# zixinz990/quadruped_landing

Measured on AMD Instinct MI355X. Metric: knot-point constraint+Jacobian evals/sec, higher is better.
Workload: dtype f64

## Files before the change

include/qln_evaluator.h:

```cpp
#ifndef QLN_EVALUATOR_H
#define QLN_EVALUATOR_H

#include <stdint.h>

#ifdef __cplusplus
extern "C" {
#endif

#define QLN_NX 15
#define QLN_NU 5
#define QLN_NZ 20
#define QLN_COST_STRIDE 41

#define QLN_OK 0
#define QLN_ERR_INVALID_ARGUMENT (-1)
#define QLN_ERR_HIP (-2)
#define QLN_ERR_NO_DEVICE (-3)
#define QLN_ERR_UNSUPPORTED (-4)

#define QLN_JAC_WRITE_CONSTANTS 1u

#define QLN_JAC_FORMAT_DENSE_BLOCKS 0
#define QLN_JAC_FORMAT_STRUCTURAL 1

// ... 118 lines not shown
                             const double* K_dot, const double* x0_dot, double* Zout_dot);
int qln_tracking_rollout_jvp_host(qln_handle* h, const double* Zref, const double* K, const double* Zout,
                                  const double* Zref_dot, const double* K_dot, const double* x0_dot, double* Zout_dot);
#define QLN_TRACK_MARG_STRIDE 8
int qln_tracking_covariance(qln_handle* h, const double* Zout, const double* K, const double* Sigma0, int32_t sigma0_batch,
                            const double* Wdiag, double* Sigma, double* marg);
int qln_tracking_covariance_host(qln_handle* h, const double* Zout, const double* K, const double* Sigma0,
                                 int32_t sigma0_batch, const double* Wdiag, double* Sigma, double* marg);
int qln_perturb_point(qln_handle* h, const qln_drop_state_sampler* s, double* Z, double sigma, double h_min, double h_max,
                      int redraw_h);
int qln_get_boundary_states(qln_handle* h, double* x0, double* xf);
int qln_set_lqr_cost(qln_handle* h, const double* Qdiag, const double* Rdiag, const double* Qfdiag, double dt,
                     int per_problem);
int qln_get_cost(qln_handle* h, double* cost_host, int32_t* cost_batch);

int qln_eval_objective_host(qln_handle* h, const double* Z, double* f);
int qln_eval_objective_gradient_host(qln_handle* h, const double* Z, double* grad);
int qln_eval_constraint_host(qln_handle* h, const double* Z, double* c);
int qln_eval_constraint_jacobian_host(qln_handle* h, const double* Z, double* vals);
int qln_eval_hessian_lagrangian_host(qln_handle* h, const double* Z, const double* sigma, const double* mu, double* hvals);
int qln_eval_hessian_lagrangian_product_host(qln_handle* h, const double* Z, const double* sigma, const double* mu,
                                             const double* v, double* y);
int qln_eval_constraint_jvp_host(qln_handle* h, const double* Z, const double* v, double* y);
int qln_eval_constraint_vjp_host(qln_handle* h, const double* Z, const double* lam, double* g);
int qln_eval_constraint_jacobian_dense_host(qln_handle* h, int32_t b, const double* Z, double* jac);

int qln_vals_alloc_placed(qln_handle* h, const double* Z, double* c, double** vals, float* ms_best);
int qln_vals_alloc_placed_budget(qln_handle* h, const double* Z, double* c, int64_t transient_bytes, double** vals, float* ms_best);
int qln_vals_placed_address_space(int64_t* retired_bytes, int64_t* cap_bytes);
int qln_vals_free_placed(qln_handle* h, double* vals);
int qln_vals_placed_info(const qln_handle* h, const double* vals, int64_t* chunk_bytes, int64_t* chunks_scanned,
                         int64_t* window_first_chunk);

int qln_time_constraint_and_jacobian(qln_handle* h, const double* Z, double* c, double* vals, uint32_t flags,
                                     int32_t warmup, int32_t iters, float* ms_each );
int qln_time_constraint_and_jacobian_total(qln_handle* h, const double* Z, double* c, double* vals, uint32_t flags,
                                           int32_t warmup, int32_t iters, float* ms_total);

#ifdef __cplusplus
}
#endif
#endif
```

quadruped_landing_amd/_lib.py:

```python
from __future__ import annotations

import ctypes as C
import os

_HERE = os.path.dirname(os.path.abspath(__file__))
LIB_PATH = os.environ.get("QLN_LIB_PATH") or os.path.join(_HERE, "csrc", "libqln_hip.so")

QLN_OK = 0
QLN_ERR_INVALID_ARGUMENT = -1
QLN_ERR_HIP = -2
QLN_ERR_NO_DEVICE = -3
QLN_ERR_UNSUPPORTED = -4
QLN_JAC_WRITE_CONSTANTS = 1
QLN_JAC_FORMAT_DENSE_BLOCKS = 0
QLN_JAC_FORMAT_STRUCTURAL = 1

NX, NU, NZ, COST_STRIDE = 15, 5, 20, 41
GN_INFO_STRIDE = 8
HESS_STEP_NNZ, HESS_TERM_NNZ = 55, 15
TRACK_NU, TRACK_P_NNZ = 4, 120
TRACK_MARG_STRIDE = 8


class QlnModel(C.Structure):
    _fields_ = [(n, C.c_double) for n in ("g", "mb", "mf", "lb", "l1", "l2")]


class QlnBatchDesc(C.Structure):
    _fields_ = [
        ("B", C.c_int32),
        ("N", C.c_int32),
        ("model", QlnModel),
        ("k_trans", C.POINTER(C.c_int32)),
        ("init_mode", C.POINTER(C.c_int32)),
        ("x0", C.POINTER(C.c_double)),
        ("xf", C.POINTER(C.c_double)),
        ("cost", C.POINTER(C.c_double)),
        ("cost_batch", C.c_int32),
        ("z_stride", C.c_int64),
        ("align", C.c_int32),
        ("jac_format", C.c_int32),
    ]


class QlnDims(C.Structure):
    _fields_ = [
# ... 98 lines not shown
    "qln_tracking_rollout_jvp": (C.c_int, [_vp, _dp, _dp, _dp, _dp, _dp, _dp, _dp]),
    "qln_tracking_rollout_jvp_host": (C.c_int, [_vp, _dp, _dp, _dp, _dp, _dp, _dp, _dp]),
    "qln_tracking_covariance": (C.c_int, [_vp, _dp, _dp, _dp, C.c_int32, _dp, _dp, _dp]),
    "qln_tracking_covariance_host": (C.c_int, [_vp, _dp, _dp, _dp, C.c_int32, _dp, _dp, _dp]),
    "qln_eval_constraint_jvp_host": (C.c_int, [_vp, _dp, _dp, _dp]),
    "qln_eval_constraint_vjp_host": (C.c_int, [_vp, _dp, _dp, _dp]),
    "qln_gauss_newton_step": (C.c_int, [_vp, _dp, _dp, _dp, C.c_int32, C.c_double, _dp, _dp, _dp]),
    "qln_eval_kinematic_constraint": (C.c_int, [_vp, _dp, _dp, _dp]),
    "qln_kinematic_bounds": (C.c_int, [_vp, C.POINTER(C.c_double), C.POINTER(C.c_double)]),
    "qln_eval_friction_cone": (C.c_int, [_vp, _dp, C.c_double, _dp, _dp]),
    "qln_constraint_violation": (C.c_int, [_vp, _dp, _dp]),
    "qln_solve_default_options": (C.c_int, [C.POINTER(QlnSolveOptions)]),
    "qln_variable_bounds": (C.c_int, [C.c_int32, C.POINTER(QlnSolveOptions), _dp, _dp]),
    "qln_solve": (C.c_int, [_vp, _dp, C.POINTER(QlnSolveOptions), _dp]),
    "qln_solve_host": (C.c_int, [_vp, _dp, C.POINTER(QlnSolveOptions), _dp]),
    "qln_initial_guess": (C.c_int, [_vp, _dp]),
    "qln_sample_drop_states": (C.c_int, [_vp, C.POINTER(QlnDropStateSampler)]),
    "qln_sample_bounded_integers": (C.c_int, [C.c_int, C.POINTER(C.c_uint64), C.POINTER(C.c_uint64), C.c_int64, C.c_int32, C.c_int32, C.c_int64,
                                            _i32p, _i64p]),
    "qln_perturb_point": (C.c_int, [_vp, C.POINTER(QlnDropStateSampler), _dp, C.c_double, C.c_double, C.c_double, C.c_int]),
    "qln_get_boundary_states": (C.c_int, [_vp, _dp, _dp]),
    "qln_set_lqr_cost": (C.c_int, [_vp, _dp, _dp, _dp, C.c_double, C.c_int]),
    "qln_get_cost": (C.c_int, [_vp, _dp, _i32p]),
    "qln_eval_objective_host": (C.c_int, [_vp, _dp, _dp]),
    "qln_eval_objective_gradient_host": (C.c_int, [_vp, _dp, _dp]),
    "qln_eval_constraint_host": (C.c_int, [_vp, _dp, _dp]),
    "qln_eval_constraint_jacobian_host": (C.c_int, [_vp, _dp, _dp]),
    "qln_eval_constraint_jacobian_dense_host": (C.c_int, [_vp, C.c_int32, _dp, _dp]),
    "qln_vals_alloc_placed": (C.c_int, [_vp, _dp, _dp, C.POINTER(_vp), C.POINTER(C.c_float)]),
    "qln_vals_free_placed": (C.c_int, [_vp, _dp]),
    "qln_vals_alloc_placed_budget": (C.c_int, [_vp, _dp, _dp, C.c_int64, C.POINTER(_vp), C.POINTER(C.c_float)]),
    "qln_vals_placed_address_space": (C.c_int, [_i64p, _i64p]),
    "qln_vals_placed_info": (C.c_int, [_vp, _dp, _i64p, _i64p, _i64p]),
    "qln_time_constraint_and_jacobian": (C.c_int, [_vp, _dp, _dp, _dp, C.c_uint32, C.c_int32, C.c_int32, C.POINTER(C.c_float)]),
    "qln_time_constraint_and_jacobian_total": (C.c_int, [_vp, _dp, _dp, _dp, C.c_uint32, C.c_int32, C.c_int32, C.POINTER(C.c_float)]),
}


def lib() -> C.CDLL:
    global _lib
    if _lib is None:
        if not os.path.exists(LIB_PATH) and not os.environ.get("QLN_LIB_PATH"):
            import shutil
            import subprocess

            csrc = os.path.join(_HERE, "csrc")
            if shutil.which("hipcc") or os.path.exists("/opt/rocm/bin/hipcc"):
                subprocess.call(["make", "-C", csrc, "libqln_hip.so"], stdout=subprocess.DEVNULL)
        if not os.path.exists(LIB_PATH):
            raise ImportError(
                f"{LIB_PATH} not found: build it with `make -C quadruped_landing_amd/csrc` "
                "(hipcc --offload-arch=gfx950).  There is no CPU fallback."
            )
        import torch

        L = C.CDLL(LIB_PATH)
        for name, (res, args) in SIGNATURES.items():
            fn = getattr(L, name)
            fn.restype = res
            fn.argtypes = args
        _lib = L
    return _lib


def check(rc: int) -> None:
    if rc != QLN_OK:
# ... 2 lines not shown
```

quadruped_landing_amd/csrc/qln_api.cpp:

```cpp
#include <hip/hip_runtime.h>

#include <algorithm>
#include <atomic>
#include <cmath>
#include <cstdio>
#include <cstdlib>
#include <cstring>
#include <initializer_list>
#include <limits>
#include <new>
#include <string>
#include <vector>

#include "../../include/qln_evaluator.h"
#include "qln_device.h"
#include "qln_hessian.h"

namespace {

thread_local std::string g_err;

int fail(int code, const std::string& msg) {
    g_err = msg;
    return code;
}

#define QLN_HIP(expr)                                                                                   \
    do {                                                                                                \
        hipError_t e_ = (expr);                                                                         \
        if (e_ != hipSuccess)                                                                           \
            return fail(QLN_ERR_HIP, std::string(#expr) + ": " + hipGetErrorString(e_));                \
    } while (0)

int64_t round_up(int64_t v, int64_t a) { return (v + a - 1) / a * a; }

int32_t hessian_nnz(int32_t N) { return QLN_HESS_STEP_NNZ * (N - 1) + QLN_HESS_TERM_NNZ; }
int64_t hessian_stride(int32_t N, int32_t align) { return round_up(hessian_nnz(N), align ? align : 16); }

constexpr bool kReturnVirtualRange = false;
constexpr uint64_t kVaCapBytes = (uint64_t)64 << 40;
std::atomic<uint64_t> g_va_retired{0};

int32_t m_nlp_of(int32_t N, int32_t kt) { return qln::row_layout(N, kt).m; }
int32_t nnz_dyn_of(int32_t N, int32_t kt, int32_t fmt) { return qln::vals_layout(N, kt, fmt).o_const; }
int32_t nnz_of(int32_t N, int32_t kt, int32_t fmt) { return qln::vals_layout(N, kt, fmt).nnz; }

int64_t tracking_k_total(const qln_dims& D) { return (int64_t)D.B * (D.N - 1) * QLN_TRACK_NU * QLN_NX; }
int64_t tracking_p_total(const qln_dims& D) { return (int64_t)D.B * D.N * QLN_TRACK_P_NNZ; }
int64_t tracking_marg_total(const qln_dims& D) { return (int64_t)D.B * D.N * QLN_TRACK_MARG_STRIDE; }

enum HostRole {
    kZ,
    kV,
    kZbar,
    kZio,
    kZdot,
    kZout,
    kGrad,
    kC,
    kMu,
    kVals,
    kF,
    kSigma,
    kHvals,
    kK,
    kKbar,
    kKdot,
    kP,
    kX0,
    kCov0,
    kCov,
    kMarg,
    kHostRoles
};

}

struct qln_handle {
    int device = 0;
    qln_model model{};
    hipStream_t stream = nullptr;
    qln::BatchParams p{};
    qln_dims dims{};
    std::vector<int32_t> k_trans, init_mode;
    std::vector<int64_t> c_off, j_off;
    qln::ProblemDesc* d_desc = nullptr;
    double* d_bnd = nullptr;
    double* d_cost = nullptr;
    int64_t h_stride = 0;
    double* staged[kHostRoles] = {};
    struct Mapped {
        double* host = nullptr;
        double* dev = nullptr;
    };
    Mapped mapped[kHostRoles];
    bool zero_copy = false;
    std::vector<double> h_vals_one;
    struct DenseMap {
        std::vector<int64_t> at, zeros;
    };
    std::vector<DenseMap> dense_map;
    struct Placed {
        char* va = nullptr;
        size_t va_size = 0;
        size_t chunk = 0;
        size_t first = 0;
        size_t scanned = 0;
        std::vector<hipMemGenericAllocationHandle_t> chunks;
        double* vals = nullptr;
    };
    std::vector<Placed> placed;
    double* solve_scratch = nullptr;
    size_t solve_scratch_n = 0;
};

namespace {

template <class T>
int upload(T** dst, const T* src, size_t n) {
    QLN_HIP(hipMalloc(reinterpret_cast<void**>(dst), std::max<size_t>(n, 1) * sizeof(T)));
    if (n) QLN_HIP(hipMemcpy(*dst, src, n * sizeof(T), hipMemcpyHostToDevice));
    return QLN_OK;
}

int64_t host_role_size(const qln_handle* h, HostRole r) {
    const qln_dims& D = h->dims;
    switch (r) {
        case kZ: case kV: case kZbar: case kZio: case kZdot: case kZout: case kGrad: return D.z_total;
        case kC: case kMu: return D.c_total;
        case kVals: return D.j_total;
        case kF: case kSigma: return D.B;
        case kHvals: return (int64_t)(D.B - 1) * h->h_stride + hessian_nnz(D.N);
        case kK: case kKbar: case kKdot: return tracking_k_total(D);
        case kP: case kCov: return tracking_p_total(D);
        case kCov0: return (int64_t)D.B * QLN_TRACK_P_NNZ;
        case kMarg: return tracking_marg_total(D);
        case kX0: return (int64_t)D.B * QLN_NX;
        case kHostRoles: break;
    }
    return 0;
}

int acquire(qln_handle* h, HostRole r, bool mapped) {
    const size_t bytes = std::max<int64_t>(host_role_size(h, r), 1) * sizeof(double);
// ... 190 lines not shown
    P.lb = d->model.lb;
    P.desc = h->d_desc;
    P.bnd = h->d_bnd;
    P.cost = h->d_cost;
    P.cost_batch = d->cost_batch;
    P.z_stride = z_stride;
    P.jac_format = fmt;
    P.kt_max = *std::max_element(d->k_trans, d->k_trans + d->B);
    h->zero_copy = (D.z_total + D.c_total + D.j_total) * (int64_t)sizeof(double) <= ((int64_t)8 << 20);
    *out = h;
    return QLN_OK;
}

static int release_placed(qln_handle::Placed& p) {
    hipError_t first = hipSuccess;
    const char* what = nullptr;
    auto note = [&](hipError_t e, const char* w) {
        if (e != hipSuccess && first == hipSuccess) {
            first = e;
            what = w;
        }
    };
    for (size_t i = 0; i < p.chunks.size(); ++i) {
        note(hipMemUnmap(p.va + (p.first + i) * p.chunk, p.chunk), "hipMemUnmap");
        note(hipMemRelease(p.chunks[i]), "hipMemRelease");
    }
    p.chunks.clear();
    if (p.va && kReturnVirtualRange) note(hipMemAddressFree(p.va, p.va_size), "hipMemAddressFree");
    p.va = nullptr;
    if (first != hipSuccess) return fail(QLN_ERR_HIP, std::string("releasing a placed buffer: ") + what + ": " + hipGetErrorString(first));
    return QLN_OK;
}

int qln_destroy(qln_handle* h) {
    if (!h) return QLN_OK;
    (void)hipSetDevice(h->device);
    int rc = QLN_OK;
    if (!h->placed.empty()) {
        if (hipError_t e = hipDeviceSynchronize(); e != hipSuccess)
            rc = fail(QLN_ERR_HIP, std::string("qln_destroy: hipDeviceSynchronize: ") + hipGetErrorString(e));
        for (auto& p : h->placed)
            if (int r = release_placed(p); r != QLN_OK && rc == QLN_OK) rc = r;
    }
    for (const qln_handle::Mapped& m : h->mapped)
        if (m.host) (void)hipHostFree(m.host);
    for (double* b : h->staged)
        if (b) (void)hipFree(b);
    void* bufs[] = {h->d_desc, h->d_bnd, h->d_cost, h->solve_scratch};
    for (void* b : bufs)
        if (b) (void)hipFree(b);
    delete h;
    return rc;
}

int qln_set_stream(qln_handle* h, void* hip_stream) {
    if (int rc = check_handle(h)) return rc;
    h->stream = reinterpret_cast<hipStream_t>(hip_stream);
    return QLN_OK;
}

int qln_synchronize(qln_handle* h) {
    if (int rc = check_handle(h)) return rc;
    if (int rc = bind_device(h)) return rc;
    QLN_HIP(hipStreamSynchronize(h->stream));
    return QLN_OK;
}

int qln_get_dims(const qln_handle* h, qln_dims* out) {
    if (int rc = check_handle(h)) return rc;
    if (!out) return fail(QLN_ERR_INVALID_ARGUMENT, "qln_get_dims: null out");
    *out = h->dims;
    return QLN_OK;
}

int qln_get_offsets(const qln_handle* h, int64_t* c_off, int64_t* j_off) {
// ... 881 lines not shown

static int time_fused(qln_handle* h, const double* Z, double* c, double* vals, int warmup, int iters, float* best) {
    hipEvent_t e0 = nullptr, e1 = nullptr;
    if (hipEventCreate(&e0) != hipSuccess || hipEventCreate(&e1) != hipSuccess) {
        if (e0) (void)hipEventDestroy(e0);
        return fail(QLN_ERR_HIP, "hipEventCreate failed");
    }
    int rc = QLN_OK;
    *best = 1e30f;
    for (int i = 0; i < warmup + iters && rc == QLN_OK; ++i) {
        (void)hipEventRecord(e0, h->stream);
        if (qln::launch_constraint_jacobian(h->p, 0, h->p.B, Z, c, vals, 0, h->stream) != hipSuccess) rc = fail(QLN_ERR_HIP, "launch failed");
        (void)hipEventRecord(e1, h->stream);
        if (rc == QLN_OK && hipEventSynchronize(e1) != hipSuccess) rc = fail(QLN_ERR_HIP, "hipEventSynchronize failed");
        float ms = 0.f;
        if (rc == QLN_OK && hipEventElapsedTime(&ms, e0, e1) != hipSuccess) rc = fail(QLN_ERR_HIP, "hipEventElapsedTime failed");
        if (rc == QLN_OK && i >= warmup) *best = std::min(*best, ms);
    }
    (void)hipEventDestroy(e0);
    (void)hipEventDestroy(e1);
    return rc;
}

int qln_vals_alloc_placed(qln_handle* h, const double* Z, double* c, double** vals, float* ms_best) {
    return qln_vals_alloc_placed_budget(h, Z, c, (int64_t)64 << 30, vals, ms_best);
}

int qln_vals_placed_address_space(int64_t* retired_bytes, int64_t* cap_bytes) {
    if (retired_bytes) *retired_bytes = (int64_t)g_va_retired.load();
    if (cap_bytes) *cap_bytes = (int64_t)kVaCapBytes;
    return QLN_OK;
}

int qln_vals_alloc_placed_budget(qln_handle* h, const double* Z, double* c, int64_t transient_bytes, double** vals, float* ms_best) {
    if (int rc = check_handle(h)) return rc;
    if (!Z || !vals) return fail(QLN_ERR_INVALID_ARGUMENT, "qln_vals_alloc_placed: null pointer");
    if (transient_bytes < 0) return fail(QLN_ERR_INVALID_ARGUMENT, "qln_vals_alloc_placed: negative transient budget");
    *vals = nullptr;
    if (int rc = bind_device(h)) return rc;
    hipMemAllocationProp prop = {};
    prop.type = hipMemAllocationTypePinned;
    prop.location.type = hipMemLocationTypeDevice;
    prop.location.id = h->device;
    size_t gran = 0;
    QLN_HIP(hipMemGetAllocationGranularity(&gran, &prop, hipMemAllocationGranularityRecommended));
    const size_t chunk = round_up((int64_t)256 << 20, (int64_t)gran);
    const size_t bytes = (size_t)h->dims.j_total * 8;
    const size_t need = (bytes + chunk - 1) / chunk;
    const size_t region = ((size_t)32 << 30) / chunk;
    const bool small = bytes < ((size_t)1 << 30);
    size_t free_b = 0, total_b = 0;
    QLN_HIP(hipMemGetInfo(&free_b, &total_b));
    const size_t budget = free_b / 10 * 9 / chunk;
    if (budget < need + 1) return fail(QLN_ERR_HIP, "qln_vals_alloc_placed: not enough free device memory");

    std::vector<hipMemGenericAllocationHandle_t> slab;
    std::vector<char> mapped;
    char* va = nullptr;
    size_t va_size = 0;
    double* scratch_c = nullptr;
    auto abandon = [&](int code) {
        (void)hipDeviceSynchronize();
        for (size_t i = 0; i < slab.size(); ++i) {
            if (i < mapped.size() && mapped[i]) (void)hipMemUnmap(va + i * chunk, chunk);
            if (slab[i]) (void)hipMemRelease(slab[i]);
        }
        if (va && kReturnVirtualRange) (void)hipMemAddressFree(va, va_size);
        if (scratch_c) (void)hipFree(scratch_c);
        return code;
    };
    auto fail_hip = [&](const char* what, hipError_t e) {
        return abandon(fail(QLN_ERR_HIP, std::string("qln_vals_alloc_placed: ") + what + ": " + hipGetErrorString(e)));
    };

    if (!c) {
        if (hipError_t e = hipMalloc(reinterpret_cast<void**>(&scratch_c), (size_t)h->dims.c_total * 8); e != hipSuccess)
            return fail_hip("hipMalloc(scratch c)", e);
        c = scratch_c;
    }
    (void)region;
    const size_t extra = ((size_t)transient_bytes + chunk - 1) / chunk;
    size_t nslab = small ? need : std::min(budget, need + extra + 1);
    if (g_va_retired.load() + (uint64_t)nslab * chunk > kVaCapBytes)
        return abandon(fail(QLN_ERR_UNSUPPORTED,
                            "qln_vals_alloc_placed: this process has retired " + std::to_string(g_va_retired.load() >> 30) +
                                " GiB of virtual address space in placed allocations (ranges are never returned: an unmapped address "
                                "must not be mapped again on this stack); the cap is " + std::to_string(kVaCapBytes >> 30) +
                                " GiB -- reuse placed buffers instead of re-allocating them, or use plain hipMalloc memory"));
    for (size_t i = 0; i < nslab; ++i) {
        hipMemGenericAllocationHandle_t hd;
        const hipError_t e = hipMemCreate(&hd, chunk, &prop, 0);
        if (e != hipSuccess) {
            if (slab.size() >= need + 1) break;
            return fail_hip("hipMemCreate", e);
        }
        slab.push_back(hd);
    }
    nslab = slab.size();
    mapped.assign(nslab, 0);
    va_size = nslab * chunk;
    {
        void* p = nullptr;
        if (hipError_t e = hipMemAddressReserve(&p, va_size, 0, nullptr, 0); e != hipSuccess) return fail_hip("hipMemAddressReserve", e);
        va = static_cast<char*>(p);
        if (!kReturnVirtualRange) g_va_retired.fetch_add((uint64_t)va_size);
    }
    for (size_t i = 0; i < nslab; ++i) {
        if (hipError_t e = hipMemMap(va + i * chunk, chunk, 0, slab[i], 0); e != hipSuccess) return fail_hip("hipMemMap", e);
        mapped[i] = 1;
    }
    {
        hipMemAccessDesc ad = {};
        ad.location = prop.location;
        ad.flags = hipMemAccessFlagsProtReadWrite;
        if (hipError_t e = hipMemSetAccess(va, va_size, &ad, 1); e != hipSuccess) return fail_hip("hipMemSetAccess", e);
    }

    size_t best_off = 0;
    float best = 1e30f;
    {
// ... 6 lines not shown
            }
            return rc;
        };
        int rc = QLN_OK;
        if (small) {
            rc = probe(0);
        } else {
            for (size_t off = 0; off + need <= nslab && rc == QLN_OK; off += 4) rc = probe(off);
            const size_t centre = best_off;
            for (int k = -3; k <= 3 && rc == QLN_OK; ++k) {
                const int64_t off = (int64_t)centre + k;
                if (k != 0 && off >= 0 && (size_t)off + need <= nslab) rc = probe((size_t)off);
            }
        }
        if (rc != QLN_OK) return abandon(rc);
    }
    if (hipError_t e = hipDeviceSynchronize(); e != hipSuccess) return fail_hip("hipDeviceSynchronize", e);
    for (size_t i = 0; i < nslab; ++i) {
        if (i >= best_off && i < best_off + need) continue;
        if (hipError_t e = hipMemUnmap(va + i * chunk, chunk); e != hipSuccess) return fail_hip("hipMemUnmap", e);
        mapped[i] = 0;
    }
    for (size_t i = 0; i < nslab; ++i) {
        if (i >= best_off && i < best_off + need) continue;
        const hipError_t e = hipMemRelease(slab[i]);
        slab[i] = nullptr;
        if (e != hipSuccess) return fail_hip("hipMemRelease", e);
    }
    if (scratch_c) {
        const hipError_t e = hipFree(scratch_c);
        scratch_c = nullptr;
        if (e != hipSuccess) return fail_hip("hipFree(scratch c)", e);
    }
    qln_handle::Placed P;
    P.chunk = chunk;
    P.va = va;
    P.va_size = va_size;
    P.first = best_off;
    P.chunks.assign(slab.begin() + (long)best_off, slab.begin() + (long)(best_off + need));
    P.vals = reinterpret_cast<double*>(va + best_off * chunk);
    P.scanned = nslab;
    h->placed.push_back(P);
    *vals = P.vals;
    if (ms_best) *ms_best = best;
    return QLN_OK;
}

int qln_vals_placed_info(const qln_handle* h, const double* vals, int64_t* chunk_bytes, int64_t* chunks_scanned,
                         int64_t* window_first_chunk) {
    if (int rc = check_handle(h)) return rc;
    for (const auto& p : h->placed)
        if (p.vals == vals) {
            if (chunk_bytes) *chunk_bytes = (int64_t)p.chunk;
            if (chunks_scanned) *chunks_scanned = (int64_t)p.scanned;
            if (window_first_chunk) *window_first_chunk = (int64_t)p.first;
            return QLN_OK;
        }
    return fail(QLN_ERR_INVALID_ARGUMENT, "qln_vals_placed_info: not a buffer of this handle");
}

int qln_vals_free_placed(qln_handle* h, double* vals) {
    if (int rc = check_handle(h)) return rc;
    if (int rc = bind_device(h)) return rc;
    for (size_t i = 0; i < h->placed.size(); ++i)
        if (h->placed[i].vals == vals) {
            QLN_HIP(hipDeviceSynchronize());
            const int rc = release_placed(h->placed[i]);
            h->placed.erase(h->placed.begin() + (long)i);
            return rc;
        }
    return fail(QLN_ERR_INVALID_ARGUMENT, "qln_vals_free_placed: not a buffer of this handle");
}


int qln_time_constraint_and_jacobian(qln_handle* h, const double* Z, double* c, double* vals, uint32_t flags, int32_t warmup,
                                     int32_t iters, float* ms_each) {
    if (int rc = check_handle(h)) return rc;
    if (!Z || !c || !ms_each || iters < 1 || warmup < 0)
        return fail(QLN_ERR_INVALID_ARGUMENT, "qln_time_constraint_and_jacobian: bad argument");
    if (int rc = check_vals(vals)) return rc;
    if (int rc = bind_device(h)) return rc;
    flags &= QLN_JAC_WRITE_CONSTANTS;
    std::vector<hipEvent_t> ev(2 * (size_t)iters, nullptr);
    int rc = QLN_OK;
    for (auto& e : ev)
        if (rc == QLN_OK && hipEventCreate(&e) != hipSuccess) rc = fail(QLN_ERR_HIP, "hipEventCreate failed");
    for (int32_t i = 0; i < warmup && rc == QLN_OK; ++i)
        if (qln::launch_constraint_jacobian(h->p, 0, h->p.B, Z, c, vals, flags, h->stream) != hipSuccess)
            rc = fail(QLN_ERR_HIP, "warmup launch failed");
    for (int32_t i = 0; i < iters && rc == QLN_OK; ++i) {
        (void)hipEventRecord(ev[2 * i], h->stream);
        if (qln::launch_constraint_jacobian(h->p, 0, h->p.B, Z, c, vals, flags, h->stream) != hipSuccess)
            rc = fail(QLN_ERR_HIP, "timed launch failed");
        (void)hipEventRecord(ev[2 * i + 1], h->stream);
    }
    if (rc == QLN_OK && hipStreamSynchronize(h->stream) != hipSuccess) rc = fail(QLN_ERR_HIP, "stream synchronize failed");
    for (int32_t i = 0; i < iters && rc == QLN_OK; ++i)
        if (hipEventElapsedTime(&ms_each[i], ev[2 * i], ev[2 * i + 1]) != hipSuccess)
            rc = fail(QLN_ERR_HIP, "hipEventElapsedTime failed");
    for (auto& e : ev)
        if (e) (void)hipEventDestroy(e);
    return rc;
}

// ... 28 lines not shown
```

quadruped_landing_amd/nlp.py:

```python
from __future__ import annotations

import ctypes as C

import numpy as np

from . import _lib
from .planar_quadruped import PlanarQuadruped

n, m = 15, 5




def num_primals(N: int) -> int:
    return n * N + m * (N - 1)


def num_duals(N: int, k_trans: int) -> int:
    return cinds(N, k_trans)[-1][-1]


def xinds(N: int):
    return [np.arange(1, n + 1) + (k - 1) * (n + m) for k in range(1, N + 1)]

# ... 85 lines not shown
    if S.shape == (n,):
        S = np.diag(S)
    if S.shape[-2:] == (n, n) and S.ndim in (2, 3):
        S = pack_covariance(S)
    if S.ndim == 1:
        S = S[None]
    if S.ndim != 2 or S.shape[1] != _lib.TRACK_P_NNZ or S.shape[0] not in (1, B):
        raise ValueError(f"Sigma0 of shape {np.shape(Sigma0)}: expected (15,), (15, 15), ({B}, 15, 15), (120,), (1, 120) or "
                         f"({B}, 120)")
    return np.ascontiguousarray(S), int(S.shape[0])


def tracking_noise(W):
    if W is None:
        return None
    return np.ascontiguousarray(np.broadcast_to(np.asarray(W, dtype=np.float64), (n,)))


def _torch():
    import torch

    return torch


def _host_ptr(a):
    return None if a is None else a.ctypes.data


JAC_FORMATS = {"dense_blocks": _lib.QLN_JAC_FORMAT_DENSE_BLOCKS, "structural": _lib.QLN_JAC_FORMAT_STRUCTURAL}


class _PlacedBuffer:

    def __init__(self, nlp, ptr: int, numel: int):
        self._nlp, self._ptr = nlp, ptr
        self.__cuda_array_interface__ = {"shape": (numel,), "typestr": "<f8", "data": (ptr, False), "version": 2}

    def __del__(self):
        h = getattr(self._nlp, "_h", None)
        if h and self._ptr:
            try:
                rc = _lib.lib().qln_vals_free_placed(h, self._ptr)
                if rc != _lib.QLN_OK:
                    import warnings

                    warnings.warn(f"qln_vals_free_placed failed ({rc}): {_lib.lib().qln_last_error().decode()}")
            except Exception:
                pass
            self._ptr = 0


class HybridNLP:

    def __init__(self, model: PlanarQuadruped, obj, init_mode, k_trans, N: int, x0, xf, *,
                 device: int = 0, z_stride: int = 0, align: int = 16, stream=None, jac_format: str = "dense_blocks",
                 exact_hessian: bool = False, matrix_free: bool = False):
        self.model = model
        self.exact_hessian = bool(exact_hessian)
        self.matrix_free = bool(matrix_free)
        if jac_format not in JAC_FORMATS:
            raise ValueError(f"jac_format must be one of {sorted(JAC_FORMATS)}")
        self.jac_format = jac_format
        self.N = int(N)
        x0 = np.asarray(x0, dtype=np.float64)
        B = x0.shape[0] if x0.ndim == 2 else 1
        self.B = B
        self.x0 = np.ascontiguousarray(np.broadcast_to(x0, (B, n)))
        self.xf = np.ascontiguousarray(np.broadcast_to(np.asarray(xf, dtype=np.float64), (B, n)))
        self.k_trans = np.ascontiguousarray(np.broadcast_to(np.asarray(k_trans, dtype=np.int32), (B,)))
        self.init_mode = np.ascontiguousarray(np.broadcast_to(np.asarray(init_mode, dtype=np.int32), (B,)))
        if obj is None:
            self.cost_batch = 1
        else:
            obj = np.ascontiguousarray(obj, dtype=np.float64)
            if obj.shape == (self.N, _lib.COST_STRIDE):
                self.cost_batch = 1
            elif obj.shape == (B, self.N, _lib.COST_STRIDE):
                self.cost_batch = B
            else:
                raise ValueError(f"obj must have shape (N,41) or (B,N,41), got {obj.shape}")
        self.obj = obj
        self.device = int(device)
# ... 64 lines not shown
    def problem_nnz_dynamic(self, b: int = 0) -> int:
        nd = C.c_int32()
        _lib.check(_lib.lib().qln_problem_nnz_dynamic(self._h, b, C.byref(nd)))
        return nd.value

    def cinds(self, b: int = 0):
        out = (C.c_int32 * 14)()
        _lib.check(_lib.lib().qln_constraint_index_ranges(self._h, b, out))
        return [(out[2 * i], out[2 * i + 1]) for i in range(7)]

    def bounds(self, b: int = 0):
        mm, _ = self.problem_dims(b)
        lb, ub = np.empty(mm), np.empty(mm)
        _lib.check(_lib.lib().qln_constraint_bounds(self._h, b, lb.ctypes.data, ub.ctypes.data))
        return lb, ub

    def jacobian_structure(self, b: int = 0):
        _, nz = self.problem_dims(b)
        rows, cols = np.zeros(nz, dtype=np.int32), np.zeros(nz, dtype=np.int32)
        ip = C.POINTER(C.c_int32)
        _lib.check(_lib.lib().qln_jacobian_structure(self._h, b, rows.ctypes.data_as(ip), cols.ctypes.data_as(ip)))
        return rows, cols

    def _dev(self):
        return _torch().device("cuda", self.device)

    def new_Z(self):
        return _torch().zeros(self.dims.z_total, dtype=_torch().float64, device=self._dev())

    def new_c(self):
        return _torch().zeros(self.dims.c_total, dtype=_torch().float64, device=self._dev())

    def new_vals(self):
        return _torch().zeros(self.dims.j_total, dtype=_torch().float64, device=self._dev())

    def placed_info(self, vals):
        a, b, c_ = C.c_int64(), C.c_int64(), C.c_int64()
        _lib.check(_lib.lib().qln_vals_placed_info(self._h, vals.data_ptr(), C.byref(a), C.byref(b), C.byref(c_)))
        return a.value, b.value, c_.value

    @staticmethod
    def placed_address_space():
        a, b = C.c_int64(), C.c_int64()
        _lib.check(_lib.lib().qln_vals_placed_address_space(C.byref(a), C.byref(b)))
        return a.value, b.value

    def new_vals_regions(self, Z, c=None, transient_gib: float = 64.0):
        t = _torch()
        self._check(Z, self.dims.z_total, "Z")
        if c is not None:
            self._check(c, self.dims.c_total, "c")
        ptr, ms = C.c_void_p(), C.c_float()
        _lib.check(_lib.lib().qln_vals_alloc_placed_budget(self._h, Z.data_ptr(), None if c is None else c.data_ptr(),
                                                           int(transient_gib * 2**30), C.byref(ptr), C.byref(ms)))
        vals = t.as_tensor(_PlacedBuffer(self, ptr.value, int(self.dims.j_total)), device=self._dev())
        return vals, float(ms.value)

    def new_vals_placed(self, Z, c, trials: int = 4, launches: int = 3, spread: bool = True, regions: bool = True):
        t = _torch()
        if regions:
            try:
                vals, ms = self.new_vals_regions(Z, c)
                return vals, [ms]
            except _lib.QlnError:
                pass
        trials = max(1, int(trials))
        nbytes = 8 * int(self.dims.j_total)
# ... 545 lines not shown
```

Baseline: 2.533 billion.

## Route default new_vals through a per-device cache of placed Jacobian buffers

Changes the default new_vals allocation so that large Jacobian value buffers (at least 1 GiB by default) go through a scanned, physically placed VMM range rather than a plain torch.zeros tensor. Ranges are kept in a per-device LRU cache and reused, because retired virtual address space cannot be remapped. The intent is that the evaluator writes into memory placed to cut write cost, with cache reuse so the expensive placement scan is paid only once. In exchange it adds allocation-time timing scans, global cache state and a free cap policy. Small buffers still fall back to hipMalloc.

After: 2.526 billion. Within noise of the previous version (-0.3%).

```diff
diff --git a/include/qln_evaluator.h b/include/qln_evaluator.h
--- a/include/qln_evaluator.h
+++ b/include/qln_evaluator.h
@@ -174,6 +174,19 @@
 int qln_vals_placed_info(const qln_handle* h, const double* vals, int64_t* chunk_bytes, int64_t* chunks_scanned,
                          int64_t* window_first_chunk);
 
+#define QLN_VALS_PLAIN 0
+#define QLN_VALS_PLACED 1
+#define QLN_VALS_PLAIN_SCAN_REFUSED 2
+int qln_vals_alloc(qln_handle* h, double** vals);
+int qln_vals_free(qln_handle* h, double* vals);
+int qln_vals_info(const qln_handle* h, const double* vals, int32_t* kind, int32_t* cache_hit, float* ms, int64_t* chunk_bytes,
+                  int64_t* chunks, int64_t* chunks_scanned, int64_t* window_first_chunk);
+int qln_vals_cache_trim(int device);
+int qln_vals_cache_stats(int device, int64_t* retired_bytes, int64_t* free_bytes, int64_t* in_use_bytes, int64_t* hits,
+                         int64_t* misses, int64_t* evicted);
+int qln_vals_cache_configure(int device, int64_t placed_min_bytes, int64_t transient_bytes, int64_t chunk_bytes,
+                             int64_t free_cap_bytes, int64_t va_cap_bytes);
+
 int qln_time_constraint_and_jacobian(qln_handle* h, const double* Z, double* c, double* vals, uint32_t flags,
                                      int32_t warmup, int32_t iters, float* ms_each );
 int qln_time_constraint_and_jacobian_total(qln_handle* h, const double* Z, double* c, double* vals, uint32_t flags,
diff --git a/quadruped_landing_amd/_lib.py b/quadruped_landing_amd/_lib.py
--- a/quadruped_landing_amd/_lib.py
+++ b/quadruped_landing_amd/_lib.py
@@ -12,6 +12,7 @@
 QLN_ERR_NO_DEVICE = -3
 QLN_ERR_UNSUPPORTED = -4
 QLN_JAC_WRITE_CONSTANTS = 1
+QLN_VALS_PLAIN, QLN_VALS_PLACED, QLN_VALS_PLAIN_SCAN_REFUSED = 0, 1, 2
 QLN_JAC_FORMAT_DENSE_BLOCKS = 0
 QLN_JAC_FORMAT_STRUCTURAL = 1
 
@@ -176,6 +177,12 @@
     "qln_vals_alloc_placed_budget": (C.c_int, [_vp, _dp, _dp, C.c_int64, C.POINTER(_vp), C.POINTER(C.c_float)]),
     "qln_vals_placed_address_space": (C.c_int, [_i64p, _i64p]),
     "qln_vals_placed_info": (C.c_int, [_vp, _dp, _i64p, _i64p, _i64p]),
+    "qln_vals_alloc": (C.c_int, [_vp, C.POINTER(_vp)]),
+    "qln_vals_free": (C.c_int, [_vp, _dp]),
+    "qln_vals_info": (C.c_int, [_vp, _dp, _i32p, _i32p, C.POINTER(C.c_float), _i64p, _i64p, _i64p, _i64p]),
+    "qln_vals_cache_trim": (C.c_int, [C.c_int]),
+    "qln_vals_cache_stats": (C.c_int, [C.c_int, _i64p, _i64p, _i64p, _i64p, _i64p, _i64p]),
+    "qln_vals_cache_configure": (C.c_int, [C.c_int, C.c_int64, C.c_int64, C.c_int64, C.c_int64, C.c_int64]),
     "qln_time_constraint_and_jacobian": (C.c_int, [_vp, _dp, _dp, _dp, C.c_uint32, C.c_int32, C.c_int32, C.POINTER(C.c_float)]),
     "qln_time_constraint_and_jacobian_total": (C.c_int, [_vp, _dp, _dp, _dp, C.c_uint32, C.c_int32, C.c_int32, C.POINTER(C.c_float)]),
 }
diff --git a/quadruped_landing_amd/csrc/qln_api.cpp b/quadruped_landing_amd/csrc/qln_api.cpp
--- a/quadruped_landing_amd/csrc/qln_api.cpp
+++ b/quadruped_landing_amd/csrc/qln_api.cpp
@@ -8,6 +8,8 @@
 #include <cstring>
 #include <initializer_list>
 #include <limits>
+#include <map>
+#include <mutex>
 #include <new>
 #include <string>
 #include <vector>
@@ -15,6 +17,7 @@
 #include "../../include/qln_evaluator.h"
 #include "qln_device.h"
 #include "qln_hessian.h"
+#include "qln_vals_cache.h"
 
 namespace {
 
@@ -74,6 +77,17 @@
     kHostRoles
 };
 
+struct PlacedRange {
+    char* va = nullptr;
+    size_t va_size = 0;
+    size_t chunk = 0;
+    size_t first = 0;
+    size_t scanned = 0;
+    std::vector<hipMemGenericAllocationHandle_t> chunks;
+    double* vals = nullptr;
+    float ms = 0.f;
+};
+
 }
 
 struct qln_handle {
@@ -100,16 +114,16 @@
         std::vector<int64_t> at, zeros;
     };
     std::vector<DenseMap> dense_map;
-    struct Placed {
-        char* va = nullptr;
-        size_t va_size = 0;
-        size_t chunk = 0;
-        size_t first = 0;
-        size_t scanned = 0;
-        std::vector<hipMemGenericAllocationHandle_t> chunks;
+    using Placed = PlacedRange;
+    std::vector<Placed> placed;
+    struct Handed {
         double* vals = nullptr;
+        int32_t kind = QLN_VALS_PLAIN;
+        int64_t id = -1;
+        bool hit = false;
+        PlacedRange range;
     };
-    std::vector<Placed> placed;
+    std::vector<Handed> handed;
     double* solve_scratch = nullptr;
     size_t solve_scratch_n = 0;
 };
@@ -366,15 +380,63 @@
     return QLN_OK;
 }
 
+struct DeviceValsCache {
+    std::mutex mu;
+    qln::ValsCachePolicy policy;
+    std::map<int64_t, PlacedRange> ranges;
+    int64_t placed_min_bytes = -1, transient_bytes = -1, chunk_bytes = -1, va_cap_bytes = -1;
+};
+static DeviceValsCache& vals_cache(int device) {
+    static std::mutex mu;
+    static auto* all = new std::map<int, DeviceValsCache*>();
+    std::lock_guard<std::mutex> lock(mu);
+    DeviceValsCache*& dc = (*all)[device];
+    if (!dc) dc = new DeviceValsCache();
+    return *dc;
+}
+
+static int drop_evicted(DeviceValsCache& dc, const std::vector<int64_t>& ids) {
+    int rc = QLN_OK;
+    for (int64_t id : ids) {
+        PlacedRange r;
+        {
+            std::lock_guard<std::mutex> lock(dc.mu);
+            auto it = dc.ranges.find(id);
+            if (it == dc.ranges.end()) continue;
+            r = std::move(it->second);
+            dc.ranges.erase(it);
+        }
+        if (int e = release_placed(r); e != QLN_OK && rc == QLN_OK) rc = e;
+    }
+    return rc;
+}
+
+static int return_to_cache(int device, int64_t id) {
+    DeviceValsCache& dc = vals_cache(device);
+    std::vector<int64_t> evicted;
+    {
+        std::lock_guard<std::mutex> lock(dc.mu);
+        if (!dc.policy.release(id, &evicted)) return fail(QLN_ERR_INVALID_ARGUMENT, "qln_vals_free: the cache does not hold this range as in use");
+    }
+    return drop_evicted(dc, evicted);
+}
+
 int qln_destroy(qln_handle* h) {
     if (!h) return QLN_OK;
     (void)hipSetDevice(h->device);
     int rc = QLN_OK;
-    if (!h->placed.empty()) {
+    if (!h->placed.empty() || !h->handed.empty()) {
         if (hipError_t e = hipDeviceSynchronize(); e != hipSuccess)
             rc = fail(QLN_ERR_HIP, std::string("qln_destroy: hipDeviceSynchronize: ") + hipGetErrorString(e));
         for (auto& p : h->placed)
             if (int r = release_placed(p); r != QLN_OK && rc == QLN_OK) rc = r;
+        for (auto& v : h->handed) {
+            if (v.kind == QLN_VALS_PLACED) {
+                if (int r = return_to_cache(h->device, v.id); r != QLN_OK && rc == QLN_OK) rc = r;
+            } else {
+                (void)hipFree(v.vals);
+            }
+        }
     }
     for (const qln_handle::Mapped& m : h->mapped)
         if (m.host) (void)hipHostFree(m.host);
@@ -1322,23 +1384,28 @@
     return QLN_OK;
 }
 
-int qln_vals_alloc_placed_budget(qln_handle* h, const double* Z, double* c, int64_t transient_bytes, double** vals, float* ms_best) {
-    if (int rc = check_handle(h)) return rc;
-    if (!Z || !vals) return fail(QLN_ERR_INVALID_ARGUMENT, "qln_vals_alloc_placed: null pointer");
-    if (transient_bytes < 0) return fail(QLN_ERR_INVALID_ARGUMENT, "qln_vals_alloc_placed: negative transient budget");
-    *vals = nullptr;
-    if (int rc = bind_device(h)) return rc;
+struct ScanOptions {
+    int64_t transient_bytes = (int64_t)64 << 30;
+    int64_t chunk_bytes = (int64_t)256 << 20;
+    int64_t placed_min_bytes = (int64_t)1 << 30;
+    uint64_t va_cap = kVaCapBytes;
+};
+
+static size_t scan_chunk_bytes(const ScanOptions& o, size_t gran) { return (size_t)round_up(o.chunk_bytes, (int64_t)gran); }
+
+static int scan_placed(qln_handle* h, const double* Z, double* c, const ScanOptions& o, PlacedRange* out) {
+    const int64_t transient_bytes = o.transient_bytes;
     hipMemAllocationProp prop = {};
     prop.type = hipMemAllocationTypePinned;
     prop.location.type = hipMemLocationTypeDevice;
     prop.location.id = h->device;
     size_t gran = 0;
     QLN_HIP(hipMemGetAllocationGranularity(&gran, &prop, hipMemAllocationGranularityRecommended));
-    const size_t chunk = round_up((int64_t)256 << 20, (int64_t)gran);
+    const size_t chunk = scan_chunk_bytes(o, gran);
     const size_t bytes = (size_t)h->dims.j_total * 8;
     const size_t need = (bytes + chunk - 1) / chunk;
     const size_t region = ((size_t)32 << 30) / chunk;
-    const bool small = bytes < ((size_t)1 << 30);
+    const bool small = bytes < (size_t)o.placed_min_bytes;
     size_t free_b = 0, total_b = 0;
     QLN_HIP(hipMemGetInfo(&free_b, &total_b));
     const size_t budget = free_b / 10 * 9 / chunk;
@@ -1371,11 +1438,11 @@
     (void)region;
     const size_t extra = ((size_t)transient_bytes + chunk - 1) / chunk;
     size_t nslab = small ? need : std::min(budget, need + extra + 1);
-    if (g_va_retired.load() + (uint64_t)nslab * chunk > kVaCapBytes)
+    if (g_va_retired.load() + (uint64_t)nslab * chunk > o.va_cap)
         return abandon(fail(QLN_ERR_UNSUPPORTED,
                             "qln_vals_alloc_placed: this process has retired " + std::to_string(g_va_retired.load() >> 30) +
                                 " GiB of virtual address space in placed allocations (ranges are never returned: an unmapped address "
-                                "must not be mapped again on this stack); the cap is " + std::to_string(kVaCapBytes >> 30) +
+                                "must not be mapped again on this stack); the cap is " + std::to_string(o.va_cap >> 30) +
                                 " GiB -- reuse placed buffers instead of re-allocating them, or use plain hipMalloc memory"));
     for (size_t i = 0; i < nslab; ++i) {
         hipMemGenericAllocationHandle_t hd;
@@ -1448,7 +1515,7 @@
         scratch_c = nullptr;
         if (e != hipSuccess) return fail_hip("hipFree(scratch c)", e);
     }
-    qln_handle::Placed P;
+    PlacedRange& P = *out;
     P.chunk = chunk;
     P.va = va;
     P.va_size = va_size;
@@ -1456,9 +1523,23 @@
     P.chunks.assign(slab.begin() + (long)best_off, slab.begin() + (long)(best_off + need));
     P.vals = reinterpret_cast<double*>(va + best_off * chunk);
     P.scanned = nslab;
+    P.ms = best;
+    return QLN_OK;
+}
+
+int qln_vals_alloc_placed_budget(qln_handle* h, const double* Z, double* c, int64_t transient_bytes, double** vals, float* ms_best) {
+    if (int rc = check_handle(h)) return rc;
+    if (!Z || !vals) return fail(QLN_ERR_INVALID_ARGUMENT, "qln_vals_alloc_placed: null pointer");
+    if (transient_bytes < 0) return fail(QLN_ERR_INVALID_ARGUMENT, "qln_vals_alloc_placed: negative transient budget");
+    *vals = nullptr;
+    if (int rc = bind_device(h)) return rc;
+    ScanOptions o;
+    o.transient_bytes = transient_bytes;
+    PlacedRange P;
+    if (int rc = scan_placed(h, Z, c, o, &P)) return rc;
     h->placed.push_back(P);
     *vals = P.vals;
-    if (ms_best) *ms_best = best;
+    if (ms_best) *ms_best = P.ms;
     return QLN_OK;
 }
 
@@ -1486,6 +1567,163 @@
             return rc;
         }
     return fail(QLN_ERR_INVALID_ARGUMENT, "qln_vals_free_placed: not a buffer of this handle");
+}
+
+
+static int scan_for_cache(qln_handle* h, const ScanOptions& o, PlacedRange* out) {
+    double* z = nullptr;
+    const size_t zbytes = (size_t)std::max<int64_t>(h->dims.z_total, 1) * 8;
+    if (hipError_t e = hipMalloc(reinterpret_cast<void**>(&z), zbytes); e != hipSuccess)
+        return fail(QLN_ERR_HIP, std::string("qln_vals_alloc: hipMalloc(transient Z): ") + hipGetErrorString(e));
+    int rc = QLN_OK;
+    if (hipError_t e = hipMemset(z, 0, zbytes); e != hipSuccess) rc = fail(QLN_ERR_HIP, std::string("qln_vals_alloc: hipMemset(transient Z): ") + hipGetErrorString(e));
+    if (rc == QLN_OK) rc = scan_placed(h, z, nullptr, o, out);
+    (void)hipFree(z);
+    return rc;
+}
+
+int qln_vals_alloc(qln_handle* h, double** vals) {
+    if (int rc = check_handle(h)) return rc;
+    if (!vals) return fail(QLN_ERR_INVALID_ARGUMENT, "qln_vals_alloc: null pointer");
+    *vals = nullptr;
+    if (int rc = bind_device(h)) return rc;
+    DeviceValsCache& dc = vals_cache(h->device);
+    ScanOptions o;
+    {
+        std::lock_guard<std::mutex> lock(dc.mu);
+        if (dc.placed_min_bytes >= 0) o.placed_min_bytes = dc.placed_min_bytes;
+        if (dc.transient_bytes >= 0) o.transient_bytes = dc.transient_bytes;
+        if (dc.chunk_bytes > 0) o.chunk_bytes = dc.chunk_bytes;
+        if (dc.va_cap_bytes >= 0) o.va_cap = (uint64_t)dc.va_cap_bytes;
+    }
+    const size_t bytes = (size_t)std::max<int64_t>(h->dims.j_total, 1) * 8;
+    qln_handle::Handed hd;
+    if (bytes >= (size_t)o.placed_min_bytes) {
+        hipMemAllocationProp prop = {};
+        prop.type = hipMemAllocationTypePinned;
+        prop.location.type = hipMemLocationTypeDevice;
+        prop.location.id = h->device;
+        size_t gran = 0;
+        QLN_HIP(hipMemGetAllocationGranularity(&gran, &prop, hipMemAllocationGranularityRecommended));
+        const size_t chunk = scan_chunk_bytes(o, gran);
+        const int64_t need = (int64_t)((bytes + chunk - 1) / chunk);
+        {
+            std::lock_guard<std::mutex> lock(dc.mu);
+            hd.id = dc.policy.acquire(need, need * (int64_t)chunk);
+            if (hd.id >= 0) hd.range = dc.ranges.at(hd.id);
+        }
+        if (hd.id >= 0) {
+            hd.hit = true;
+        } else if (scan_for_cache(h, o, &hd.range) == QLN_OK) {
+            std::lock_guard<std::mutex> lock(dc.mu);
+            hd.id = dc.policy.insert((int64_t)hd.range.chunks.size(), (int64_t)(hd.range.chunks.size() * hd.range.chunk));
+            dc.ranges[hd.id] = hd.range;
+        }
+        if (hd.id >= 0) {
+            hd.kind = QLN_VALS_PLACED;
+            hd.vals = hd.range.vals;
+        } else {
+            hd.kind = QLN_VALS_PLAIN_SCAN_REFUSED;
+            hd.range = PlacedRange();
+        }
+    }
+    auto give_back = [&](int code) {
+        if (hd.kind == QLN_VALS_PLACED) {
+            (void)hipDeviceSynchronize();
+            (void)return_to_cache(h->device, hd.id);
+        } else if (hd.vals) {
+            (void)hipFree(hd.vals);
+        }
+        return code;
+    };
+    if (!hd.vals)
+        if (hipError_t e = hipMalloc(reinterpret_cast<void**>(&hd.vals), bytes); e != hipSuccess)
+            return fail(QLN_ERR_HIP, std::string("qln_vals_alloc: hipMalloc: ") + hipGetErrorString(e));
+    hipError_t e = hipMemsetAsync(hd.vals, 0, bytes, h->stream);
+    if (e == hipSuccess) e = hipStreamSynchronize(h->stream);
+    if (e != hipSuccess) return give_back(fail(QLN_ERR_HIP, std::string("qln_vals_alloc: clearing the buffer: ") + hipGetErrorString(e)));
+    h->handed.push_back(hd);
+    *vals = hd.vals;
+    return QLN_OK;
+}
+
+int qln_vals_free(qln_handle* h, double* vals) {
+    if (int rc = check_handle(h)) return rc;
+    if (int rc = bind_device(h)) return rc;
+    for (size_t i = 0; i < h->handed.size(); ++i)
+        if (h->handed[i].vals == vals) {
+            const qln_handle::Handed hd = h->handed[i];
+            if (hd.kind != QLN_VALS_PLACED) {
+                h->handed.erase(h->handed.begin() + (long)i);
+                QLN_HIP(hipFree(hd.vals));
+                return QLN_OK;
+            }
+            QLN_HIP(hipDeviceSynchronize());
+            h->handed.erase(h->handed.begin() + (long)i);
+            return return_to_cache(h->device, hd.id);
+        }
+    return fail(QLN_ERR_INVALID_ARGUMENT, "qln_vals_free: not a buffer of this handle");
+}
+
+int qln_vals_info(const qln_handle* h, const double* vals, int32_t* kind, int32_t* cache_hit, float* ms, int64_t* chunk_bytes,
+                  int64_t* chunks, int64_t* chunks_scanned, int64_t* window_first_chunk) {
+    if (int rc = check_handle(h)) return rc;
+    for (const auto& v : h->handed)
+        if (v.vals == vals) {
+            if (kind) *kind = v.kind;
+            if (cache_hit) *cache_hit = v.hit ? 1 : 0;
+            if (ms) *ms = v.range.ms;
+            if (chunk_bytes) *chunk_bytes = (int64_t)v.range.chunk;
+            if (chunks) *chunks = (int64_t)v.range.chunks.size();
+            if (chunks_scanned) *chunks_scanned = (int64_t)v.range.scanned;
+            if (window_first_chunk) *window_first_chunk = (int64_t)v.range.first;
+            return QLN_OK;
+        }
+    return fail(QLN_ERR_INVALID_ARGUMENT, "qln_vals_info: not a buffer of this handle");
+}
+
+int qln_vals_cache_trim(int device) {
+    if (device < 0) return fail(QLN_ERR_INVALID_ARGUMENT, "qln_vals_cache_trim: bad device ordinal");
+    DeviceValsCache& dc = vals_cache(device);
+    std::vector<int64_t> evicted;
+    {
+        std::lock_guard<std::mutex> lock(dc.mu);
+        dc.policy.trim(&evicted);
+    }
+    if (evicted.empty()) return QLN_OK;
+    int prev = 0;
+    QLN_HIP(hipGetDevice(&prev));
+    QLN_HIP(hipSetDevice(device));
+    const int rc = drop_evicted(dc, evicted);
+    (void)hipSetDevice(prev);
+    return rc;
+}
+
+int qln_vals_cache_stats(int device, int64_t* retired_bytes, int64_t* free_bytes, int64_t* in_use_bytes, int64_t* hits,
+                         int64_t* misses, int64_t* evicted) {
+    if (device < 0) return fail(QLN_ERR_INVALID_ARGUMENT, "qln_vals_cache_stats: bad device ordinal");
+    DeviceValsCache& dc = vals_cache(device);
+    std::lock_guard<std::mutex> lock(dc.mu);
+    if (retired_bytes) *retired_bytes = (int64_t)g_va_retired.load();
+    if (free_bytes) *free_bytes = dc.policy.free_bytes();
+    if (in_use_bytes) *in_use_bytes = dc.policy.in_use_bytes();
+    if (hits) *hits = (int64_t)dc.policy.counters().hits;
+    if (misses) *misses = (int64_t)dc.policy.counters().misses;
+    if (evicted) *evicted = (int64_t)dc.policy.counters().evicted;
+    return QLN_OK;
+}
+
+int qln_vals_cache_configure(int device, int64_t placed_min_bytes, int64_t transient_bytes, int64_t chunk_bytes,
+                             int64_t free_cap_bytes, int64_t va_cap_bytes) {
+    if (device < 0) return fail(QLN_ERR_INVALID_ARGUMENT, "qln_vals_cache_configure: bad device ordinal");
+    DeviceValsCache& dc = vals_cache(device);
+    std::lock_guard<std::mutex> lock(dc.mu);
+    dc.placed_min_bytes = placed_min_bytes;
+    dc.transient_bytes = transient_bytes;
+    dc.chunk_bytes = chunk_bytes;
+    dc.va_cap_bytes = va_cap_bytes;
+    dc.policy.set_free_cap(free_cap_bytes);
+    return QLN_OK;
 }
 
 
diff --git a/quadruped_landing_amd/csrc/qln_vals_cache.h b/quadruped_landing_amd/csrc/qln_vals_cache.h
--- /dev/null
+++ b/quadruped_landing_amd/csrc/qln_vals_cache.h
@@ -0,0 +1,98 @@
+#pragma once
+
+#include <algorithm>
+#include <cstddef>
+#include <cstdint>
+#include <vector>
+
+namespace qln {
+
+class ValsCachePolicy {
+public:
+    struct Entry {
+        int64_t id = 0;
+        int64_t chunks = 0, bytes = 0;
+        bool in_use = false;
+        uint64_t freed_at = 0;
+    };
+    struct Counters {
+        uint64_t hits = 0, misses = 0, inserted = 0, evicted = 0;
+        int64_t evicted_bytes = 0;
+    };
+
+    int64_t acquire(int64_t chunks, int64_t bytes) {
+        largest_request_ = std::max(largest_request_, bytes);
+        Entry* best = nullptr;
+        for (Entry& e : entries_)
+            if (!e.in_use && e.chunks == chunks && e.bytes == bytes && (!best || e.freed_at < best->freed_at)) best = &e;
+        if (!best) {
+            ++counters_.misses;
+            return -1;
+        }
+        ++counters_.hits;
+        best->in_use = true;
+        return best->id;
+    }
+
+    int64_t insert(int64_t chunks, int64_t bytes) {
+        Entry e;
+        e.id = next_id_++;
+        e.chunks = chunks;
+        e.bytes = bytes;
+        e.in_use = true;
+        entries_.push_back(e);
+        ++counters_.inserted;
+        return e.id;
+    }
+
+    bool release(int64_t id, std::vector<int64_t>* evicted) {
+        Entry* e = find(id);
+        if (!e || !e->in_use) return false;
+        e->in_use = false;
+        e->freed_at = ++clock_;
+        enforce(free_cap(), evicted);
+        return true;
+    }
+
+    void trim(std::vector<int64_t>* evicted) { enforce(-1, evicted); }
+
+    void set_free_cap(int64_t bytes) { cap_ = bytes; }
+    int64_t free_cap() const { return cap_ < 0 ? largest_request_ : cap_; }
+
+    int64_t free_bytes() const { return sum(false); }
+    int64_t in_use_bytes() const { return sum(true); }
+    const Counters& counters() const { return counters_; }
+    const std::vector<Entry>& entries() const { return entries_; }
+
+private:
+    Entry* find(int64_t id) {
+        for (Entry& e : entries_)
+            if (e.id == id) return &e;
+        return nullptr;
+    }
+    int64_t sum(bool in_use) const {
+        int64_t s = 0;
+        for (const Entry& e : entries_)
+            if (e.in_use == in_use) s += e.bytes;
+        return s;
+    }
+    void enforce(int64_t cap, std::vector<int64_t>* evicted) {
+        for (;;) {
+            size_t oldest = entries_.size();
+            for (size_t i = 0; i < entries_.size(); ++i)
+                if (!entries_[i].in_use && (oldest == entries_.size() || entries_[i].freed_at < entries_[oldest].freed_at)) oldest = i;
+            if (oldest == entries_.size() || (cap >= 0 && free_bytes() <= cap)) return;
+            ++counters_.evicted;
+            counters_.evicted_bytes += entries_[oldest].bytes;
+            if (evicted) evicted->push_back(entries_[oldest].id);
+            entries_.erase(entries_.begin() + (std::ptrdiff_t)oldest);
+        }
+    }
+
+    std::vector<Entry> entries_;
+    Counters counters_;
+    int64_t next_id_ = 1, largest_request_ = 0, cap_ = -1;
+    uint64_t clock_ = 0;
+};
+
+}
diff --git a/quadruped_landing_amd/nlp.py b/quadruped_landing_amd/nlp.py
--- a/quadruped_landing_amd/nlp.py
+++ b/quadruped_landing_amd/nlp.py
@@ -141,6 +141,8 @@
 
 class _PlacedBuffer:
 
+    _free = "qln_vals_free_placed"
+
     def __init__(self, nlp, ptr: int, numel: int):
         self._nlp, self._ptr = nlp, ptr
         self.__cuda_array_interface__ = {"shape": (numel,), "typestr": "<f8", "data": (ptr, False), "version": 2}
@@ -149,14 +151,19 @@
         h = getattr(self._nlp, "_h", None)
         if h and self._ptr:
             try:
-                rc = _lib.lib().qln_vals_free_placed(h, self._ptr)
+                rc = getattr(_lib.lib(), self._free)(h, self._ptr)
                 if rc != _lib.QLN_OK:
                     import warnings
 
-                    warnings.warn(f"qln_vals_free_placed failed ({rc}): {_lib.lib().qln_last_error().decode()}")
+                    warnings.warn(f"{self._free} failed ({rc}): {_lib.lib().qln_last_error().decode()}")
             except Exception:
                 pass
             self._ptr = 0
+
+
+class _ValsBuffer(_PlacedBuffer):
+
+    _free = "qln_vals_free"
 
 
 class HybridNLP:
@@ -287,7 +294,27 @@
         return _torch().zeros(self.dims.c_total, dtype=_torch().float64, device=self._dev())
 
     def new_vals(self):
-        return _torch().zeros(self.dims.j_total, dtype=_torch().float64, device=self._dev())
+        ptr = C.c_void_p()
+        _lib.check(_lib.lib().qln_vals_alloc(self._h, C.byref(ptr)))
+        return _torch().as_tensor(_ValsBuffer(self, ptr.value, int(self.dims.j_total)), device=self._dev())
+
+    def vals_info(self, vals):
+        k, hit, ms = C.c_int32(), C.c_int32(), C.c_float()
+        a, n_, s_, f_ = C.c_int64(), C.c_int64(), C.c_int64(), C.c_int64()
+        _lib.check(_lib.lib().qln_vals_info(self._h, vals.data_ptr(), C.byref(k), C.byref(hit), C.byref(ms), C.byref(a),
+                                            C.byref(n_), C.byref(s_), C.byref(f_)))
+        return dict(kind=k.value, cache_hit=bool(hit.value), ms=float(ms.value), chunk_bytes=a.value, chunks=n_.value,
+                    chunks_scanned=s_.value, window_first_chunk=f_.value)
+
+    @staticmethod
+    def vals_cache_stats(device: int = 0):
+        v = [C.c_int64() for _ in range(6)]
+        _lib.check(_lib.lib().qln_vals_cache_stats(int(device), *[C.byref(x) for x in v]))
+        return dict(zip(("retired_bytes", "free_bytes", "in_use_bytes", "hits", "misses", "evicted"), (x.value for x in v)))
+
+    @staticmethod
+    def vals_cache_trim(device: int = 0):
+        _lib.check(_lib.lib().qln_vals_cache_trim(int(device)))
 
     def placed_info(self, vals):
         a, b, c_ = C.c_int64(), C.c_int64(), C.c_int64()
```
